# bhansconnect/burn-ppo

Hardware: AMD Instinct MI355X
Metric: env-steps/sec (rollout+GAE+PPO update) at 1/2/4/8 MI355X; steps-to-475-return CartPole (higher is better)
Workload: dtype f32

## Files before the change

### burn-ppo_amd/csrc/k_update.hip

```cpp
#include <algorithm>
#include <cstdlib>
#include "bppo_internal.h"
#include "bppo_mlp64.h"

namespace bppo {

constexpr int STAT_BLOCKS = 1024;

enum { M_PL = 0, M_VL, M_H, M_KL, M_CF, M_V, M_R, M_VE, M_VE2, M_VEMAX, M_N, NUM_M };

constexpr int ADAM_CHUNK = 4096;
struct AdamTensor { int off, len; float c1, c2; };
struct AdamArgs {
    float *params, *grad, *m1, *m2;
    double *part;
    AdamTensor t[32];
    int blk0[33];
    int nt;
    float lr, max_norm, eps, inv_world;
};
constexpr int SLAB_GROUPS = 32;

struct MbArgs {
    const float *obs, *logp, *adv, *ret, *val;
// ... 431 lines not shown
            float lh = 0.0f, vv = 0.0f;
            const float *hr = B.T2 + c * RS;
            const float2 *pv = S.PV[h];
#pragma unroll 16
            for (int k = 0; k < H; k++) {
                const float hk = hr[k];
                const float2 w = pv[k];
                lh = __builtin_fmaf(hk, w.x, lh);
                vv = __builtin_fmaf(hk, w.y, vv);
            }
            const float lx = __shfl_xor(lh, 32, 64);
            const float l0 = h ? lx : lh, l1 = h ? lh : lx;
            MB_STAMP(9);
            const float lg0 = __fadd_rn(l0, S.bp[0]), lg1 = __fadd_rn(l1, S.bp[1]), v = __fadd_rn(vv, S.bv[0]);
            const float mx = lg0 > lg1 ? lg0 : lg1;
            const float eh = S.expf(__fsub_rn(h ? lg1 : lg0, mx));
            const float eo = __shfl_xor(eh, 32, 64);
            const float e0 = h ? eo : eh, e1 = h ? eh : eo;
            const float lse = S.logf(__fadd_rn(e0, e1));
            const float ls0 = __fsub_rn(__fsub_rn(lg0, mx), lse);
            const float ls1 = __fsub_rn(__fsub_rn(lg1, mx), lse);
            const float ph = S.expf(h ? ls1 : ls0);
            const float po = __shfl_xor(ph, 32, 64);
            const float p0 = h ? po : ph, p1 = h ? ph : po;
          if (h == 0) {
            const float An = __fdiv_rn(__fsub_rn(A, mean), denom);
            const float Hn = -__fadd_rn(__fmul_rn(p0, ls0), __fmul_rn(p1, ls1));
            const float newlp = a == 1 ? ls1 : ls0;
            const float log_ratio = __fsub_rn(newlp, olp);
            const float ratio = S.expf(log_ratio);
            const float na = -An;
            const float pl1 = __fmul_rn(na, ratio);
            const float rc = ratio < g.lo ? g.lo : (ratio > g.hi ? g.hi : ratio);
            const float pl2 = __fmul_rn(na, rc);
            const bool rhs = pl1 < pl2;
            const float pl = rhs ? pl2 : pl1;
            float vl, dvl;
            if (g.clip_value) {
                const float dlt = __fsub_rn(v, ov);
                const float dc = dlt < -g.ceps ? -g.ceps : (dlt > g.ceps ? g.ceps : dlt);
                const float vc = __fadd_rn(ov, dc);
                const float q1 = __fmul_rn(__fsub_rn(v, R), __fsub_rn(v, R));
                const float q2 = __fmul_rn(__fsub_rn(vc, R), __fsub_rn(vc, R));
                if (q1 < q2) { vl = q2; dvl = (dlt >= -g.ceps && dlt <= g.ceps) ? 2.0f * __fsub_rn(vc, R) : 0.0f; }
                else { vl = q1; dvl = 2.0f * __fsub_rn(v, R); }
            } else {
                vl = __fmul_rn(__fsub_rn(v, R), __fsub_rn(v, R));
                dvl = 2.0f * __fsub_rn(v, R);
            }
            const float g_ratio = (!rhs || (ratio >= g.lo && ratio <= g.hi)) ? -An * g.inv_mb : 0.0f;
            const float g_lr = g_ratio * ratio;
            const float ec = g.ent_coef * g.inv_mb;
            float dl0 = g_lr * ((a == 0 ? 1.0f : 0.0f) - p0) + ec * p0 * (ls0 + Hn);
            float dl1 = g_lr * ((a == 1 ? 1.0f : 0.0f) - p1) + ec * p1 * (ls1 + Hn);
            float dv = g.value_coef * 0.5f * g.inv_mb * dvl;
            if (!valid) { dl0 = dl1 = dv = 0.0f; }
            else {
                const float ve = fabsf(__fsub_rn(v, R));
                m_pl += pl; m_vl += vl; m_h += Hn; m_kl += (ratio - 1.0f) - log_ratio;
                m_cf += fabsf(ratio - 1.0f) > g.ceps ? 1.0f : 0.0f;
                m_v += v; m_r += R; m_ve += ve; m_ve2 += ve * ve; m_vemax = fmaxf(m_vemax, ve);
                m_n += 1.0f;
            }
            gbp0 += dl0; gbp1 += dl1; gbv += dv;
            B.dl[c * 4 + 0] = dl0; B.dl[c * 4 + 1] = dl1; B.dl[c * 4 + 2] = dv; B.dl[c * 4 + 3] = 0.0f;
          }
        }
        wave_sync();
        MB_STAMP(10);
        MB_STAMP(4);
#pragma unroll 4
        for (int q = 0; q < 16; q++) {
            const int row = cd_row(q, h);
            const float d0 = B.dl[row * 4], d1 = B.dl[row * 4 + 1], dvr = B.dl[row * 4 + 2];
#pragma unroll
            for (int ct = 0; ct < 2; ct++) {
                const float hv = B.T2[row * RS + c + 32 * ct];
                gP0[ct] = __builtin_fmaf(hv, d0, gP0[ct]);
                gP1[ct] = __builtin_fmaf(hv, d1, gP1[ct]);
                gV[ct] = __builtin_fmaf(hv, dvr, gV[ct]);
            }
        }
#pragma unroll
        for (int ct = 0; ct < 2; ct++)
#pragma unroll
            for (int q = 0; q < 16; q++) acc[ct][q] = 0.0f;
        {
            const float a0 = B.dl[c * 4 + h], a1 = B.dl[c * 4 + 2 + h];
#pragma unroll
            for (int ct = 0; ct < 2; ct++) {
                acc[ct] = __builtin_amdgcn_mfma_f32_32x32x2f32(a0, h ? wpk1[ct] : wpk0[ct], acc[ct], 0, 0, 0);
                acc[ct] = __builtin_amdgcn_mfma_f32_32x32x2f32(a1, h ? 0.0f : wvk[ct], acc[ct], 0, 0, 0);
            }
        }
#pragma unroll
        for (int q = 0; q < 16; q++) {
#pragma unroll
            for (int ct = 0; ct < 2; ct++) {
                const int ad = cd_row(q, h) * RS + c + 32 * ct;
                const float dz = B.T2[ad] > 0.0f ? acc[ct][q] : 0.0f;
                gb1[ct] += dz;
                B.T2[ad] = dz;
            }
            if ((q & 3) == 3) __builtin_amdgcn_sched_barrier(0);
        }
        wave_sync();
        MB_STAMP(5);
#pragma unroll
        for (int jt = 0; jt < 2; jt++)
#pragma unroll
            for (int q = 0; q < 16; q++) acc[jt][q] = 0.0f;
        __builtin_amdgcn_s_setprio(3);
#pragma unroll 4
        for (int s2 = 0; s2 < 16; s2++) {
#pragma unroll
            for (int u = 0; u < 2; u++) {
                const int s = 2 * s2 + u;
                const float av = B.T2[c * RS + 2 * s + h];
                const float bw0 = S.W1[c * RS + 2 * s + h], bw1 = S.W1[(c + 32) * RS + 2 * s + h];
                acc[0] = __builtin_amdgcn_mfma_f32_32x32x2f32(av, bw0, acc[0], 0, 0, 0);
                acc[1] = __builtin_amdgcn_mfma_f32_32x32x2f32(av, bw1, acc[1], 0, 0, 0);
            }
            const int rr = (2 * s2 + h) * RS;
            const float a0 = B.T1[rr + c], a1 = B.T1[rr + c + 32];
            const float z0 = B.T2[rr + c], z1 = B.T2[rr + c + 32];
            dW1[0][0] = __builtin_amdgcn_mfma_f32_32x32x2f32(a0, z0, dW1[0][0], 0, 0, 0);
            dW1[0][1] = __builtin_amdgcn_mfma_f32_32x32x2f32(a0, z1, dW1[0][1], 0, 0, 0);
            dW1[1][0] = __builtin_amdgcn_mfma_f32_32x32x2f32(a1, z0, dW1[1][0], 0, 0, 0);
            dW1[1][1] = __builtin_amdgcn_mfma_f32_32x32x2f32(a1, z1, dW1[1][1], 0, 0, 0);
        }
        __builtin_amdgcn_s_setprio(0);
        MB_STAMP(6);
#pragma unroll
        for (int q = 0; q < 16; q++) {
            const int row = cd_row(q, h);
            float xr[5];
#pragma unroll
            for (int d = 0; d < 5; d++) xr[d] = B.X[row * 5 + d];
#pragma unroll
            for (int jt = 0; jt < 2; jt++) {
                const float dzv = B.T1[row * RS + c + 32 * jt] > 0.0f ? acc[jt][q] : 0.0f;
                gb0[jt] += dzv;
#pragma unroll
                for (int d = 0; d < 5; d++) gW0[d][jt] = __builtin_fmaf(xr[d], dzv, gW0[d][jt]);
            }
            if ((q & 3) == 3) __builtin_amdgcn_sched_barrier(0);
        }
        wave_sync();
        MB_STAMP(7);
    }
#pragma unroll
    for (int ct = 0; ct < 2; ct++) {
        gb0[ct] += __shfl_xor(gb0[ct], 32, 64); gb1[ct] += __shfl_xor(gb1[ct], 32, 64);
        gP0[ct] += __shfl_xor(gP0[ct], 32, 64); gP1[ct] += __shfl_xor(gP1[ct], 32, 64);
        gV[ct] += __shfl_xor(gV[ct], 32, 64);
#pragma unroll
        for (int d = 0; d < 5; d++) gW0[d][ct] += __shfl_xor(gW0[d][ct], 32, 64);
    }
    const int W_ = g.np + NUM_M;
    __syncthreads();
    float *row = smem + (size_t)wv * W_;
    if (h == 0) {
#pragma unroll
        for (int ct = 0; ct < 2; ct++) {
            const int k = c + 32 * ct;
#pragma unroll
            for (int d = 0; d < 5; d++) row[O.w0 + d * H + k] = gW0[d][ct];
            row[O.b0 + k] = gb0[ct];
            row[O.b1 + k] = gb1[ct];
            row[O.wp + 2 * k] = gP0[ct];
            row[O.wp + 2 * k + 1] = gP1[ct];
            row[O.wv + k] = gV[ct];
        }
    }
#pragma unroll
    for (int it = 0; it < 2; it++)
#pragma unroll
        for (int jt = 0; jt < 2; jt++)
#pragma unroll
            for (int q = 0; q < 16; q++)
                row[O.w1 + ((q & 3) + 8 * (q >> 2) + 4 * h + 32 * it) * H + c + 32 * jt] = dW1[it][jt][q];
    const float s_bp0 = wave_sum(gbp0), s_bp1 = wave_sum(gbp1), s_bv = wave_sum(gbv);
    const float s_pl = wave_sum(m_pl), s_vl = wave_sum(m_vl), s_h = wave_sum(m_h);
    const float s_kl = wave_sum(m_kl), s_cf = wave_sum(m_cf), s_v = wave_sum(m_v);
    const float s_r = wave_sum(m_r), s_ve = wave_sum(m_ve), s_ve2 = wave_sum(m_ve2);
    const float s_mx = wave_max(m_vemax), s_n = wave_sum(m_n);
    if (lane == 0) {
        row[O.bp] = s_bp0; row[O.bp + 1] = s_bp1; row[O.bv] = s_bv;
        float *mm = row + g.np;
        mm[M_PL] = s_pl; mm[M_VL] = s_vl; mm[M_H] = s_h; mm[M_KL] = s_kl; mm[M_CF] = s_cf;
        mm[M_V] = s_v; mm[M_R] = s_r; mm[M_VE] = s_ve; mm[M_VE2] = s_ve2; mm[M_VEMAX] = s_mx;
        mm[M_N] = s_n;
    }
    __syncthreads();
    for (int p = tid; p < W_; p += blockDim.x) {
        float acc = smem[p];
        if (p == g.np + M_VEMAX) {
            for (int w = 1; w < WAVES; w++) acc = fmaxf(acc, smem[(size_t)w * W_ + p]);
        } else {
            for (int w = 1; w < WAVES; w++) acc += smem[(size_t)w * W_ + p];
        }
        g.slab[(size_t)blockIdx.x * W_ + p] = acc;
    }
#ifdef BPPO_MB_STAMPS
    MB_STAMP(8);
    if (lane == 0)
        for (int k = 0; k < MB_NSEG; k++) g.stamps[(size_t)gwave * MB_NSEG + k] = st_acc[k];
#endif
}

namespace mmf {
constexpr int H = 64, TR = 32, WS = 68;
typedef __bf16 bf16x8_t __attribute__((ext_vector_type(8)));
typedef short s16x4_t __attribute__((ext_vector_type(4)));
typedef short s16x8_t __attribute__((ext_vector_type(8)));
struct Params {
    uint64_t exp2tab[32];
    double linvc[16], llogc[16];
    float W0[6 * H];
    float b1[H];
    float4 Wh[H];
    float bp[2], bv[2];
    float2 PV[2][H];
    __bf16 W1[3][H * H];
    __device__ __forceinline__ float expf(float x) const { return bppo_math::expf_glibc_tab(x, exp2tab); }
    __device__ __forceinline__ float logf(float x) const { return bppo_math::logf_glibc_tab(x, linvc, llogc); }
};
constexpr int MET_STRIDE = 20;
template <bool EXACT_FWD>
struct Wave {
    float X[TR * 5];
    union {
        float T[TR * WS];
        __bf16 Z[EXACT_FWD ? 4 : 3 * H * TR];
    };
    float dl[TR * 4];
    float met[TR * MET_STRIDE];
};
enum { MT_PL = 0, MT_VL, MT_H, MT_KL, MT_CF, MT_V, MT_R, MT_VE, MT_VE2, MT_VEMAX, MT_N, MT_BP0, MT_BP1, MT_BV };
constexpr int WAVES = 8;
constexpr size_t W1F_BYTES = H * H * sizeof(float);
template <bool EXACT_FWD>
constexpr size_t lds_tiles() { return sizeof(Params) + (EXACT_FWD ? W1F_BYTES : 0) + WAVES * sizeof(Wave<EXACT_FWD>); }
static_assert(lds_tiles<false>() <= 160 * 1024 && lds_tiles<true>() <= 160 * 1024,
              "split minibatch kernel LDS over the gfx950 limit");
static_assert(sizeof(Params) % 16 == 0 && offsetof(Params, W1) % 16 == 0 && sizeof(Wave<false>) % 16 == 0 &&
              sizeof(Wave<true>) % 16 == 0, "LDS images 16-B aligned");
__device__ __forceinline__ int w1_swz(int j1) { return (((j1 >> 1) & 1) << 2) | (((j1 >> 2) & 1) << 1) | ((j1 >> 3) & 1); }
__device__ __forceinline__ int w1_at(int j1, int j2) { return j1 * H + ((((j2 >> 3) ^ w1_swz(j1)) << 3) | (j2 & 7)); }
__device__ __forceinline__ int z_swz(int j2) { return ((j2 >> 2) & 7) ^ (((j2 >> 1) & 1) << 2); }
__device__ __forceinline__ int z_at(int j2, int row) { return j2 * TR + ((((row >> 2) ^ z_swz(j2)) << 2) | (row & 3)); }
__device__ __forceinline__ s16x4_t lds_tr4(const __bf16 *p) {
    return __builtin_amdgcn_ds_read_tr16_b64_v4i16((__attribute__((address_space(3))) s16x4_t *)p);
}
__device__ __forceinline__ bf16x8_t cat8(s16x4_t lo, s16x4_t hi) {
    return __builtin_bit_cast(bf16x8_t, (s16x8_t)__builtin_shufflevector(lo, hi, 0, 1, 2, 3, 4, 5, 6, 7));
}
struct Split8 { bf16x8_t p[3]; };
typedef __bf16 bf16x2_t __attribute__((ext_vector_type(2)));
__device__ __forceinline__ uint32_t pk_bf16(float a, float b) {
    uint32_t u = __builtin_bit_cast(uint32_t, bf16x2_t{(__bf16)a, (__bf16)b});
    asm("" : "+v"(u));
    return u;
}
union Pieces8 { bf16x8_t v; uint32_t u[4]; };
__device__ __forceinline__ Split8 split8(const float (&x)[8]) {
#ifdef BPPO_SPLIT8_SCALAR
    Split8 t;
#pragma unroll
    for (int j = 0; j < 8; j++) {
        const __bf16 a = (__bf16)x[j];
        const float r = x[j] - (float)a;
        const __bf16 b = (__bf16)r;
        t.p[0][j] = a; t.p[1][j] = b; t.p[2][j] = (__bf16)(r - (float)b);
    }
    return t;
#endif
    Pieces8 p0, p1, p2;
#pragma unroll
    for (int j = 0; j < 4; j++) {
        const float xa = x[2 * j], xb = x[2 * j + 1];
        const uint32_t A = pk_bf16(xa, xb);
        const float ra = xa - __uint_as_float(A << 16), rb = xb - __uint_as_float(A & 0xffff0000u);
        const uint32_t B = pk_bf16(ra, rb);
        const float sa = ra - __uint_as_float(B << 16), sb = rb - __uint_as_float(B & 0xffff0000u);
        p0.u[j] = A; p1.u[j] = B; p2.u[j] = pk_bf16(sa, sb);
    }
    Split8 s;
    s.p[0] = p0.v; s.p[1] = p1.v; s.p[2] = p2.v;
    return s;
}
__device__ __forceinline__ float relu_bits(float v) {
    const int b = __float_as_int(v);
    return __int_as_float(b > 0 ? b : 0);
}
__device__ __forceinline__ void mfma6(f32x16_t &acc, const Split8 &a, const Split8 &b) {
    acc = __builtin_amdgcn_mfma_f32_32x32x16_bf16(a.p[2], b.p[0], acc, 0, 0, 0);
    acc = __builtin_amdgcn_mfma_f32_32x32x16_bf16(a.p[1], b.p[1], acc, 0, 0, 0);
    acc = __builtin_amdgcn_mfma_f32_32x32x16_bf16(a.p[0], b.p[2], acc, 0, 0, 0);
    acc = __builtin_amdgcn_mfma_f32_32x32x16_bf16(a.p[1], b.p[0], acc, 0, 0, 0);
    acc = __builtin_amdgcn_mfma_f32_32x32x16_bf16(a.p[0], b.p[1], acc, 0, 0, 0);
    acc = __builtin_amdgcn_mfma_f32_32x32x16_bf16(a.p[0], b.p[0], acc, 0, 0, 0);
}
__device__ __forceinline__ Split8 w1_row_pieces(const __bf16 (*W1)[H * H], int j1, int j2) {
    Split8 s;
    const int off = w1_at(j1, j2);
#pragma unroll
    for (int p = 0; p < 3; p++) s.p[p] = *reinterpret_cast<const bf16x8_t *>(W1[p] + off);
    return s;
}
__device__ __forceinline__ Split8 w1_tr_pieces(const __bf16 (*W1)[H * H], int base, const int (&off)[2]) {
    Split8 s;
#pragma unroll
    for (int p = 0; p < 3; p++) s.p[p] = cat8(lds_tr4(W1[p] + base + off[0]), lds_tr4(W1[p] + base + off[1]));
    return s;
}
template <bool EXACT_FWD>
__device__ __forceinline__ void load_params_split(Params &S, float *W1f, const float *__restrict__ P) {
    constexpr CpOffsets O = cp_offsets<64, 2>();
    for (int i = threadIdx.x; i < 6 * H; i += blockDim.x) S.W0[i] = i < 5 * H ? P[O.w0 + i] : P[O.b0 + i - 5 * H];
    for (int t = threadIdx.x; t < H * H / 8; t += blockDim.x) {
        const int j1 = t >> 3, j2 = (t & 7) * 8;
        float w[8];
#pragma unroll
        for (int j = 0; j < 8; j++) w[j] = P[O.w1 + 8 * t + j];
        const Split8 sp = split8(w);
        const int off = w1_at(j1, j2);
#pragma unroll
        for (int p = 0; p < 3; p++) *reinterpret_cast<bf16x8_t *>(S.W1[p] + off) = sp.p[p];
        if (EXACT_FWD) {
#pragma unroll
            for (int j = 0; j < 8; j++) W1f[8 * t + j] = w[j];
        }
    }
    for (int i = threadIdx.x; i < H; i += blockDim.x) {
        S.b1[i] = P[O.b1 + i];
        S.Wh[i] = make_float4(P[O.wp + 2 * i], P[O.wp + 2 * i + 1], P[O.wv + i], 0.0f);
        if (EXACT_FWD) {
            S.PV[0][i] = make_float2(P[O.wp + 2 * i], P[O.wv + i]);
            S.PV[1][i] = make_float2(P[O.wp + 2 * i + 1], P[O.wv + i]);
        }
    }
    if (threadIdx.x < 32) S.exp2tab[threadIdx.x] = bppo_math::kExp2fTab[threadIdx.x];
    if (threadIdx.x < 16) {
        S.linvc[threadIdx.x] = bppo_math::kLogfInvc[threadIdx.x];
        S.llogc[threadIdx.x] = bppo_math::kLogfLogc[threadIdx.x];
    }
    if (threadIdx.x < 2) S.bp[threadIdx.x] = P[O.bp + threadIdx.x];
    if (threadIdx.x == 0) S.bv[0] = P[O.bv];
}
}

template <bool EXACT_FWD>
__global__ void __launch_bounds__(512, 2) k_minibatch_split(MbArgs g) {
    using namespace mmf;
    using mmb::cd_row;
    constexpr CpOffsets O = cp_offsets<64, 2>();
    extern __shared__ __attribute__((aligned(16))) float smem[];
    Params &S = *reinterpret_cast<Params *>(smem);
    float *W1f = smem + sizeof(Params) / 4;
    const int tid = threadIdx.x, lane = tid & 63, wv = tid >> 6;
    Wave<EXACT_FWD> &B = reinterpret_cast<Wave<EXACT_FWD> *>(smem + (sizeof(Params) + (EXACT_FWD ? W1F_BYTES : 0)) / 4)[wv];
    load_params_split<EXACT_FWD>(S, W1f, g.params);
    __syncthreads();
#ifdef BPPO_MB_STAMPS
    unsigned long long st_acc[MB_NSEG] = {}, st_prev;
    asm volatile("s_memtime %0\n\ts_waitcnt lgkmcnt(0)" : "=s"(st_prev)::"memory");
#endif

    const int c = lane & 31, h = lane >> 5;
    const int gwave = blockIdx.x * WAVES + wv, nwaves = gridDim.x * WAVES;
    const float mean = g.mb_stats[0], denom = g.mb_stats[1] + 1e-8f;
    int w1tr[2][2];
    {
        const int q = (lane >> 2) & 3, p = lane & 3, gq = (lane >> 4) & 1;
#pragma unroll
        for (int ct = 0; ct < 2; ct++)
#pragma unroll
            for (int e = 0; e < 2; e++) w1tr[ct][e] = w1_at(4 * h + 8 * e + q, 32 * ct + 16 * gq + 4 * p);
    }
    f32x16_t dW1[2][2];
#pragma unroll
    for (int i = 0; i < 2; i++)
#pragma unroll
        for (int j = 0; j < 2; j++)
#pragma unroll
            for (int q = 0; q < 16; q++) dW1[i][j][q] = 0.0f;
    float gW0[5][2], gb0[2] = {0, 0}, gb1[2] = {0, 0}, gP0[2] = {0, 0}, gP1[2] = {0, 0}, gV[2] = {0, 0};
#pragma unroll
    for (int d = 0; d < 5; d++) gW0[d][0] = gW0[d][1] = 0.0f;
    if (h == 0) {
        float4 *mp = reinterpret_cast<float4 *>(B.met + c * MET_STRIDE);
        mp[0] = make_float4(0, 0, 0, 0); mp[1] = make_float4(0, 0, 0, 0);
        mp[2] = make_float4(0, -INFINITY, 0, 0); mp[3] = make_float4(0, 0, 0, 0);
    }

    const uint32_t stride = (uint32_t)nwaves * TR;
    auto idx_of = [&](uint32_t b) -> uint32_t {
        const uint32_t rr = b + c;
        return (h == 0 && rr < g.n) ? g.perm[g.start + rr] : 0xFFFFFFFFu;
    };
    RowData nxt;
    uint32_t idx_next = idx_of((uint32_t)gwave * TR + stride);
    nxt = load_row(g, idx_of((uint32_t)gwave * TR));
    __builtin_amdgcn_s_waitcnt(0);
    for (uint32_t base = (uint32_t)gwave * TR; base < g.n; base += stride) {
        const uint32_t r = base + c;
        const bool valid = h == 0 && r < g.n;
        const RowData cur = row_used(nxt, g.clip_value);
        int ln_ = lane;
        asm volatile("" : "+v"(ln_));
        const int c = ln_ & 31, h = ln_ >> 5;
        const uint32_t idx_after = idx_of(base + 2 * stride);
        nxt = load_row(g, idx_next);
        idx_next = idx_after;
        const int a = cur.a;
        const float olp = cur.olp, A = cur.A, R = cur.R, ov = cur.ov;
        if (h == 0) {
#pragma unroll
            for (int d = 0; d < 5; d++) B.X[c * 5 + d] = cur.x(d);
        }
        wave_sync();
        MB_STAMP(0);
        float xs[3];
#pragma unroll
        for (int s = 0; s < 3; s++) xs[s] = (s == 2 && h == 1) ? 1.0f : B.X[c * 5 + 2 * s + h];
        f32x16_t h2[2];
#pragma unroll
        for (int ct = 0; ct < 2; ct++)
#pragma unroll
            for (int q = 0; q < 16; q++) h2[ct][q] = 0.0f;
        __builtin_amdgcn_s_setprio(3);
#pragma unroll
        for (int it = 0; it < 2; it++) {
            f32x16_t a1;
#pragma unroll
            for (int q = 0; q < 16; q++) a1[q] = 0.0f;
#pragma unroll
            for (int s = 0; s < 3; s++)
                a1 = __builtin_amdgcn_mfma_f32_32x32x2f32(S.W0[(2 * s + h) * H + c + 32 * it], xs[s], a1, 0, 0, 0);
            if (EXACT_FWD) {
#pragma unroll
                for (int q = 0; q < 16; q++) B.T[(cd_row(q, h) + 32 * it) * TR + c] = relu_bits(a1[q]);
                continue;
            }
#pragma unroll
            for (int s2 = 0; s2 < 2; s2++) {
                float v8[8];
#pragma unroll
                for (int j = 0; j < 8; j++) v8[j] = relu_bits(a1[8 * s2 + j]);
                const Split8 Af = split8(v8);
#pragma unroll
                for (int ct = 0; ct < 2; ct++)
                    mfma6(h2[ct], Af, w1_tr_pieces(S.W1, (32 * it + 16 * s2) * H, w1tr[ct]));
                __builtin_amdgcn_sched_barrier(0);
            }
        }
        if (EXACT_FWD) {
            wave_sync();
#pragma unroll 4
            for (int s = 0; s < 32; s++) {
                const float av = B.T[(2 * s + h) * TR + c];
                const float bv0 = W1f[(2 * s + h) * H + c], bv1 = W1f[(2 * s + h) * H + c + 32];
                h2[0] = __builtin_amdgcn_mfma_f32_32x32x2f32(av, bv0, h2[0], 0, 0, 0);
                h2[1] = __builtin_amdgcn_mfma_f32_32x32x2f32(av, bv1, h2[1], 0, 0, 0);
            }
        }
        __builtin_amdgcn_s_setprio(0);
        MB_STAMP(1);
        if (EXACT_FWD) wave_sync();
#pragma unroll
        for (int ct = 0; ct < 2; ct++)
#pragma unroll
            for (int q = 0; q < 16; q++) {
                const float v = h2[ct][q] + S.b1[c + 32 * ct];
                B.T[cd_row(q, h) * WS + c + 32 * ct] = relu_bits(v);
            }
        wave_sync();
        MB_STAMP(2);
        float l0, l1, vv;
        if (EXACT_FWD) {
            float lh = 0.0f, vc = 0.0f;
            const float *hr = B.T + c * WS;
            const float2 *pv = S.PV[h];
#pragma unroll 2
            for (int k = 0; k < H; k += 4) {
                const float4 x = *reinterpret_cast<const float4 *>(hr + k);
                const float xs4[4] = {x.x, x.y, x.z, x.w};
#pragma unroll
                for (int u = 0; u < 4; u++) {
                    const float2 w = pv[k + u];
                    lh = __builtin_fmaf(xs4[u], w.x, lh);
                    vc = __builtin_fmaf(xs4[u], w.y, vc);
                }
            }
            const float lx = __shfl_xor(lh, 32, 64);
            l0 = h ? lx : lh; l1 = h ? lh : lx; vv = vc;
        } else {
            float pa[3] = {0, 0, 0}, pb[3] = {0, 0, 0};
            const float *hr = B.T + c * WS + 32 * h;
#pragma unroll
            for (int k = 0; k < 32; k += 4) {
                const float4 x = *reinterpret_cast<const float4 *>(hr + k);
                const float4 w0 = S.Wh[32 * h + k], w1 = S.Wh[32 * h + k + 1];
                const float4 w2 = S.Wh[32 * h + k + 2], w3 = S.Wh[32 * h + k + 3];
                pa[0] = __builtin_fmaf(x.x, w0.x, pa[0]); pa[1] = __builtin_fmaf(x.x, w0.y, pa[1]); pa[2] = __builtin_fmaf(x.x, w0.z, pa[2]);
                pb[0] = __builtin_fmaf(x.y, w1.x, pb[0]); pb[1] = __builtin_fmaf(x.y, w1.y, pb[1]); pb[2] = __builtin_fmaf(x.y, w1.z, pb[2]);
                pa[0] = __builtin_fmaf(x.z, w2.x, pa[0]); pa[1] = __builtin_fmaf(x.z, w2.y, pa[1]); pa[2] = __builtin_fmaf(x.z, w2.z, pa[2]);
                pb[0] = __builtin_fmaf(x.w, w3.x, pb[0]); pb[1] = __builtin_fmaf(x.w, w3.y, pb[1]); pb[2] = __builtin_fmaf(x.w, w3.z, pb[2]);
            }
            float t0 = pa[0] + pb[0], t1 = pa[1] + pb[1], t2 = pa[2] + pb[2];
            t0 += __shfl_xor(t0, 32, 64); t1 += __shfl_xor(t1, 32, 64); t2 += __shfl_xor(t2, 32, 64);
            l0 = t0; l1 = t1; vv = t2;
        }
        MB_STAMP(3);
        {
            const float lg0 = __fadd_rn(l0, S.bp[0]), lg1 = __fadd_rn(l1, S.bp[1]), v = __fadd_rn(vv, S.bv[0]);
            const float mx = lg0 > lg1 ? lg0 : lg1;
            const float eh = S.expf(__fsub_rn(h ? lg1 : lg0, mx));
            const float eo = __shfl_xor(eh, 32, 64);
            const float e0 = h ? eo : eh, e1 = h ? eh : eo;
            const float lse = S.logf(__fadd_rn(e0, e1));
            const float ls0 = __fsub_rn(__fsub_rn(lg0, mx), lse);
            const float ls1 = __fsub_rn(__fsub_rn(lg1, mx), lse);
            const float ph = S.expf(h ? ls1 : ls0);
            const float po = __shfl_xor(ph, 32, 64);
            const float p0 = h ? po : ph, p1 = h ? ph : po;
          if (h == 0) {
            const float An = __fdiv_rn(__fsub_rn(A, mean), denom);
            const float Hn = -__fadd_rn(__fmul_rn(p0, ls0), __fmul_rn(p1, ls1));
            const float newlp = a == 1 ? ls1 : ls0;
            const float log_ratio = __fsub_rn(newlp, olp);
            const float ratio = S.expf(log_ratio);
            const float na = -An;
            const float pl1 = __fmul_rn(na, ratio);
            const float rc = ratio < g.lo ? g.lo : (ratio > g.hi ? g.hi : ratio);
            const float pl2 = __fmul_rn(na, rc);
            const bool rhs = pl1 < pl2;
            const float pl = rhs ? pl2 : pl1;
            float vl, dvl;
            if (g.clip_value) {
                const float dlt = __fsub_rn(v, ov);
                const float dc = dlt < -g.ceps ? -g.ceps : (dlt > g.ceps ? g.ceps : dlt);
                const float vc = __fadd_rn(ov, dc);
                const float q1 = __fmul_rn(__fsub_rn(v, R), __fsub_rn(v, R));
                const float q2 = __fmul_rn(__fsub_rn(vc, R), __fsub_rn(vc, R));
                if (q1 < q2) { vl = q2; dvl = (dlt >= -g.ceps && dlt <= g.ceps) ? 2.0f * __fsub_rn(vc, R) : 0.0f; }
                else { vl = q1; dvl = 2.0f * __fsub_rn(v, R); }
            } else {
                vl = __fmul_rn(__fsub_rn(v, R), __fsub_rn(v, R));
                dvl = 2.0f * __fsub_rn(v, R);
            }
            const float g_ratio = (!rhs || (ratio >= g.lo && ratio <= g.hi)) ? -An * g.inv_mb : 0.0f;
            const float g_lr = g_ratio * ratio;
            const float ec = g.ent_coef * g.inv_mb;
            float dl0 = g_lr * ((a == 0 ? 1.0f : 0.0f) - p0) + ec * p0 * (ls0 + Hn);
            float dl1 = g_lr * ((a == 1 ? 1.0f : 0.0f) - p1) + ec * p1 * (ls1 + Hn);
            float dv = g.value_coef * 0.5f * g.inv_mb * dvl;
            if (!valid) { dl0 = dl1 = dv = 0.0f; }
            else {
                const float ve = fabsf(__fsub_rn(v, R));
                float4 *mp = reinterpret_cast<float4 *>(B.met + c * MET_STRIDE);
                float4 m0 = mp[0], m1 = mp[1], m2 = mp[2], m3 = mp[3];
                m0.x += pl; m0.y += vl; m0.z += Hn; m0.w += (ratio - 1.0f) - log_ratio;
                m1.x += fabsf(ratio - 1.0f) > g.ceps ? 1.0f : 0.0f;
                m1.y += v; m1.z += R; m1.w += ve; m2.x += ve * ve; m2.y = fmaxf(m2.y, ve);
                m2.z += 1.0f; m2.w += dl0; m3.x += dl1; m3.y += dv;
                mp[0] = m0; mp[1] = m1; mp[2] = m2; mp[3] = m3;
            }
            *reinterpret_cast<float4 *>(B.dl + c * 4) = make_float4(dl0, dl1, dv, 0.0f);
          }
        }
        wave_sync();
        MB_STAMP(4);
#pragma unroll 4
        for (int q = 0; q < 16; q++) {
            const int row = cd_row(q, h);
            const float4 d = *reinterpret_cast<const float4 *>(B.dl + row * 4);
#pragma unroll
            for (int ct = 0; ct < 2; ct++) {
                const float hv = B.T[row * WS + c + 32 * ct];
                gP0[ct] = __builtin_fmaf(hv, d.x, gP0[ct]);
                gP1[ct] = __builtin_fmaf(hv, d.y, gP1[ct]);
                gV[ct] = __builtin_fmaf(hv, d.z, gV[ct]);
            }
        }
        f32x16_t acc[2];
#pragma unroll
        for (int ct = 0; ct < 2; ct++)
#pragma unroll
            for (int q = 0; q < 16; q++) acc[ct][q] = 0.0f;
        {
            const float a0 = B.dl[c * 4 + h], a1 = B.dl[c * 4 + 2 + h];
#pragma unroll
            for (int ct = 0; ct < 2; ct++) {
                const float4 w = S.Wh[c + 32 * ct];
                acc[ct] = __builtin_amdgcn_mfma_f32_32x32x2f32(a0, h ? w.y : w.x, acc[ct], 0, 0, 0);
                acc[ct] = __builtin_amdgcn_mfma_f32_32x32x2f32(a1, h ? 0.0f : w.z, acc[ct], 0, 0, 0);
            }
        }
        if (EXACT_FWD) {
#pragma unroll
            for (int q = 0; q < 16; q++) {
#pragma unroll
                for (int ct = 0; ct < 2; ct++) {
                    const int ad = cd_row(q, h) * WS + c + 32 * ct;
                    const float dz = B.T[ad] > 0.0f ? acc[ct][q] : 0.0f;
                    gb1[ct] += dz;
                    B.T[ad] = dz;
                }
                if ((q & 3) == 3) __builtin_amdgcn_sched_barrier(0);
            }
        } else {
#pragma unroll
            for (int q = 0; q < 16; q++)
#pragma unroll
                for (int ct = 0; ct < 2; ct++) {
                    acc[ct][q] = B.T[cd_row(q, h) * WS + c + 32 * ct] > 0.0f ? acc[ct][q] : 0.0f;
                    gb1[ct] += acc[ct][q];
                }
            wave_sync();
#pragma unroll
            for (int s2 = 0; s2 < 2; s2++)
#pragma unroll
                for (int t = 0; t < 2; t++) {
                    float z[8];
#pragma unroll
                    for (int j = 0; j < 8; j++) z[j] = acc[t][8 * s2 + j];
                    const Split8 P = split8(z);
#pragma unroll
                    for (int p = 0; p < 3; p++) {
                        const uint4 u = __builtin_bit_cast(uint4, P.p[p]);
                        *reinterpret_cast<uint2 *>(B.Z + p * H * TR + z_at(c + 32 * t, 16 * s2 + 4 * h)) = make_uint2(u.x, u.y);
                        *reinterpret_cast<uint2 *>(B.Z + p * H * TR + z_at(c + 32 * t, 16 * s2 + 8 + 4 * h)) = make_uint2(u.z, u.w);
                    }
                    __builtin_amdgcn_sched_barrier(0);
                }
        }
        MB_STAMP(5);
        __builtin_amdgcn_s_setprio(3);
        f32x16_t h1[2];
#pragma unroll
        for (int jt = 0; jt < 2; jt++)
#pragma unroll
            for (int q = 0; q < 16; q++) h1[jt][q] = 0.0f;
#pragma unroll
        for (int s = 0; s < 3; s++) {
            const float xv = (s == 2 && h == 1) ? 1.0f : B.X[c * 5 + 2 * s + h];
#pragma unroll
            for (int jt = 0; jt < 2; jt++)
                h1[jt] = __builtin_amdgcn_mfma_f32_32x32x2f32(xv, S.W0[(2 * s + h) * H + c + 32 * jt], h1[jt], 0, 0, 0);
        }
        uint32_t m1 = 0;
#pragma unroll
        for (int jt = 0; jt < 2; jt++)
#pragma unroll
            for (int q = 0; q < 16; q++) {
                h1[jt][q] = relu_bits(h1[jt][q]);
                const uint32_t hb = __float_as_uint(h1[jt][q]);
                m1 |= (hb < 1u ? hb : 1u) << (q + 16 * jt);
            }
        MB_STAMP(6);
#pragma unroll
        for (int s2 = 0; s2 < 2; s2++) {
            Split8 Bz[2];
#pragma unroll
            for (int t = 0; t < 2; t++) {
                if (EXACT_FWD) {
                    float z[8];
#pragma unroll
                    for (int j = 0; j < 8; j++) z[j] = B.T[cd_row(8 * s2 + j, h) * WS + c + 32 * t];
                    Bz[t] = split8(z);
                } else {
#pragma unroll
                    for (int p = 0; p < 3; p++) {
                        const uint2 lo = *reinterpret_cast<const uint2 *>(B.Z + p * H * TR + z_at(c + 32 * t, 16 * s2 + 4 * h));
                        const uint2 hi = *reinterpret_cast<const uint2 *>(B.Z + p * H * TR + z_at(c + 32 * t, 16 * s2 + 8 + 4 * h));
                        Bz[t].p[p] = __builtin_bit_cast(bf16x8_t, make_uint4(lo.x, lo.y, hi.x, hi.y));
                    }
                }
            }
#pragma unroll
            for (int it = 0; it < 2; it++) {
                float u[8];
#pragma unroll
                for (int j = 0; j < 8; j++) u[j] = h1[it][8 * s2 + j];
                const Split8 Ah = split8(u);
#pragma unroll
                for (int jt = 0; jt < 2; jt++) mfma6(dW1[it][jt], Ah, Bz[jt]);
                __builtin_amdgcn_sched_barrier(0);
            }
        }
        wave_sync();
        MB_STAMP(7);
        f32x16_t dz1[2];
#pragma unroll
        for (int ct = 0; ct < 2; ct++)
#pragma unroll
            for (int q = 0; q < 16; q++) dz1[ct][q] = 0.0f;
#pragma unroll
        for (int ks = 0; ks < 4; ks++) {
            Split8 Az;
            if (EXACT_FWD) {
                const float *zr = B.T + c * WS + 16 * ks + 8 * h;
                const float4 z0 = *reinterpret_cast<const float4 *>(zr), z1 = *reinterpret_cast<const float4 *>(zr + 4);
                const float zz[8] = {z0.x, z0.y, z0.z, z0.w, z1.x, z1.y, z1.z, z1.w};
                Az = split8(zz);
            } else {
                const int q = (lane >> 2) & 3, pp = lane & 3, gq = (lane >> 4) & 1;
#pragma unroll
                for (int p = 0; p < 3; p++)
                    Az.p[p] = cat8(lds_tr4(B.Z + p * H * TR + z_at(16 * ks + 8 * h + q, 16 * gq + 4 * pp)),
                                   lds_tr4(B.Z + p * H * TR + z_at(16 * ks + 8 * h + 4 + q, 16 * gq + 4 * pp)));
            }
#pragma unroll
            for (int ct = 0; ct < 2; ct++)
                mfma6(dz1[ct], Az, w1_row_pieces(S.W1, c + 32 * ct, 16 * ks + 8 * h));
            __builtin_amdgcn_sched_barrier(0);
        }
        __builtin_amdgcn_s_setprio(0);
        MB_STAMP(8);
#pragma unroll
        for (int q = 0; q < 16; q++) {
            const int row = cd_row(q, h);
            float xr[5];
#pragma unroll
            for (int d = 0; d < 5; d++) xr[d] = B.X[row * 5 + d];
#pragma unroll
            for (int jt = 0; jt < 2; jt++) {
                const int mk = (int)(m1 << (31 - (q + 16 * jt))) >> 31;
                const float dzv = __int_as_float(__float_as_int(dz1[jt][q]) & mk);
                gb0[jt] += dzv;
#pragma unroll
                for (int d = 0; d < 5; d++) gW0[d][jt] = __builtin_fmaf(xr[d], dzv, gW0[d][jt]);
            }
            if ((q & 3) == 3) __builtin_amdgcn_sched_barrier(0);
        }
        wave_sync();
        MB_STAMP(9);
    }
#pragma unroll
    for (int ct = 0; ct < 2; ct++) {
        gb0[ct] += __shfl_xor(gb0[ct], 32, 64); gb1[ct] += __shfl_xor(gb1[ct], 32, 64);
        gP0[ct] += __shfl_xor(gP0[ct], 32, 64); gP1[ct] += __shfl_xor(gP1[ct], 32, 64);
        gV[ct] += __shfl_xor(gV[ct], 32, 64);
#pragma unroll
        for (int d = 0; d < 5; d++) gW0[d][ct] += __shfl_xor(gW0[d][ct], 32, 64);
    }
    float mt[14];
#pragma unroll
    for (int k = 0; k < 14; k++) mt[k] = h == 0 ? B.met[c * MET_STRIDE + k] : (k == MT_VEMAX ? -INFINITY : 0.0f);
    const int W_ = g.np + NUM_M;
    __syncthreads();
    float *row = smem + (size_t)wv * W_;
    if (h == 0) {
#pragma unroll
        for (int ct = 0; ct < 2; ct++) {
            const int k = c + 32 * ct;
#pragma unroll
            for (int d = 0; d < 5; d++) row[O.w0 + d * H + k] = gW0[d][ct];
            row[O.b0 + k] = gb0[ct];
            row[O.b1 + k] = gb1[ct];
            row[O.wp + 2 * k] = gP0[ct];
            row[O.wp + 2 * k + 1] = gP1[ct];
            row[O.wv + k] = gV[ct];
        }
    }
#pragma unroll
    for (int it = 0; it < 2; it++)
#pragma unroll
        for (int jt = 0; jt < 2; jt++)
#pragma unroll
            for (int q = 0; q < 16; q++)
                row[O.w1 + ((q & 3) + 8 * (q >> 2) + 4 * h + 32 * it) * H + c + 32 * jt] = dW1[it][jt][q];
    float st[14];
#pragma unroll
    for (int k = 0; k < 14; k++) st[k] = k == MT_VEMAX ? wave_max(mt[k]) : wave_sum(mt[k]);
    if (lane == 0) {
        row[O.bp] = st[MT_BP0]; row[O.bp + 1] = st[MT_BP1]; row[O.bv] = st[MT_BV];
        float *mm = row + g.np;
        static_assert(MT_PL == M_PL && MT_VEMAX == M_VEMAX && MT_N == M_N, "metric slots");
#pragma unroll
        for (int k = 0; k <= MT_N; k++) mm[k] = st[k];
    }
    __syncthreads();
    for (int p = tid; p < W_; p += blockDim.x) {
        float a2 = smem[p];
        if (p == g.np + M_VEMAX) {
            for (int w = 1; w < WAVES; w++) a2 = fmaxf(a2, smem[(size_t)w * W_ + p]);
        } else {
            for (int w = 1; w < WAVES; w++) a2 += smem[(size_t)w * W_ + p];
        }
        g.slab[(size_t)blockIdx.x * W_ + p] = a2;
    }
#ifdef BPPO_MB_STAMPS
    MB_STAMP(10);
    if (lane == 0)
        for (int k = 0; k < MB_NSEG; k++) g.stamps[(size_t)gwave * MB_NSEG + k] = st_acc[k];
#endif
}

constexpr int SLAB1_COLS = 16;
__global__ void __launch_bounds__(SLAB1_COLS * SLAB_GROUPS) k_slab_reduce1(const float *__restrict__ slab, int rows,
                                                                           int width, float *__restrict__ grad,
                                                                           float *__restrict__ vemax_local) {
    __shared__ double part[SLAB_GROUPS][SLAB1_COLS];
    const int c = threadIdx.x % SLAB1_COLS, g = threadIdx.x / SLAB1_COLS;
    const int p = blockIdx.x * SLAB1_COLS + c;
    const bool live = p < width, is_max = p == width - NUM_M + M_VEMAX;
    const int per = (rows + SLAB_GROUPS - 1) / SLAB_GROUPS;
    if (live) {
        const int w0 = g * per, w1 = min(rows, w0 + per);
        double s = is_max ? -INFINITY : 0.0;
#pragma unroll 8
        for (int w = w0; w < w1; w++) {
            const double v = slab[(size_t)w * width + p];
            s = is_max ? fmax(s, v) : s + v;
        }
        part[g][c] = s;
    }
    __syncthreads();
    if (g == 0 && live) {
        double s = is_max ? -INFINITY : 0.0;
        for (int q = 0; q < SLAB_GROUPS; q++) s = is_max ? fmax(s, part[q][c]) : s + part[q][c];
        grad[p] = (float)s;
        if (is_max) *vemax_local = (float)s;
    }
}

__device__ __forceinline__ int adam_tensor_of(const AdamArgs &a, int b) {
    int t = 0;
    while (t + 1 < a.nt && a.blk0[t + 1] <= b) t++;
    return t;
}
__global__ void __launch_bounds__(256) k_adam_norm(AdamArgs a) {
    __shared__ double red[256];
    const int ti = adam_tensor_of(a, blockIdx.x);
    const AdamTensor T = a.t[ti];
    const int i0 = (blockIdx.x - a.blk0[ti]) * ADAM_CHUNK, i1 = min(T.len, i0 + ADAM_CHUNK);
    double ss = 0.0;
    for (int i = i0 + threadIdx.x; i < i1; i += blockDim.x) {
        const float gi = a.grad[T.off + i] * a.inv_world;
        ss += (double)gi * (double)gi;
    }
    red[threadIdx.x] = ss;
    __syncthreads();
    for (int st = 128; st > 0; st >>= 1) {
        if (threadIdx.x < st) red[threadIdx.x] += red[threadIdx.x + st];
        __syncthreads();
    }
    if (threadIdx.x == 0) a.part[blockIdx.x] = red[0];
}
__global__ void __launch_bounds__(256) k_adam(AdamArgs a) {
    __shared__ double tot;
    const int ti = adam_tensor_of(a, blockIdx.x);
    const AdamTensor T = a.t[ti];
    if (threadIdx.x == 0) {
        double s = 0.0;
        for (int b = a.blk0[ti]; b < a.blk0[ti + 1]; b++) s += a.part[b];
        tot = s;
    }
    __syncthreads();
    const int i0 = (blockIdx.x - a.blk0[ti]) * ADAM_CHUNK, i1 = min(T.len, i0 + ADAM_CHUNK);
    const float norm = (float)sqrt(tot);
    const float scale = norm > a.max_norm ? __fdiv_rn(a.max_norm, norm) : 1.0f;
    const bool clip = norm > a.max_norm;
    const float b1 = 0.9f, b2 = 0.999f, f1 = 1.0f - 0.9f, f2 = 1.0f - 0.999f;
    for (int i = i0 + threadIdx.x; i < i1; i += blockDim.x) {
        float gi = a.grad[T.off + i] * a.inv_world;
        if (clip) gi = __fmul_rn(gi, scale);
        const float m1 = __fadd_rn(__fmul_rn(a.m1[T.off + i], b1), __fmul_rn(gi, f1));
        const float m2 = __fadd_rn(__fmul_rn(a.m2[T.off + i], b2), __fmul_rn(__fmul_rn(gi, gi), f2));
        a.m1[T.off + i] = m1;
        a.m2[T.off + i] = m2;
        const float m1c = __fdiv_rn(m1, T.c1), m2c = __fdiv_rn(m2, T.c2);
        const float upd = __fdiv_rn(m1c, __fadd_rn(sqrtf(m2c), a.eps));
        a.params[T.off + i] = __fsub_rn(a.params[T.off + i], __fmul_rn(upd, a.lr));
    }
}

constexpr int ADAM1_THREADS = 1024;
__global__ void __launch_bounds__(ADAM1_THREADS) k_adam1(AdamArgs a, const float *gtail, const float *mb_stats,
                                                         int nm, float *metric_dst) {
    __shared__ double red[256];
    const AdamTensor T = a.t[blockIdx.x];
    if (threadIdx.x < 256) {
        double ss = 0.0;
#pragma unroll 4
        for (int i = threadIdx.x; i < T.len; i += 256) {
            const float gi = a.grad[T.off + i] * a.inv_world;
            ss += (double)gi * (double)gi;
        }
        red[threadIdx.x] = ss;
    }
    __syncthreads();
    for (int st = 128; st > 0; st >>= 1) {
        if (threadIdx.x < st) red[threadIdx.x] += red[threadIdx.x + st];
        __syncthreads();
    }
    const double tot = red[0];
    const float norm = (float)sqrt(tot);
    const float scale = norm > a.max_norm ? __fdiv_rn(a.max_norm, norm) : 1.0f;
    const bool clip = norm > a.max_norm;
    const float b1 = 0.9f, b2 = 0.999f, f1 = 1.0f - 0.9f, f2 = 1.0f - 0.999f;
#pragma unroll 2
    for (int i = threadIdx.x; i < T.len; i += ADAM1_THREADS) {
        float gi = a.grad[T.off + i] * a.inv_world;
        if (clip) gi = __fmul_rn(gi, scale);
        const float m1 = __fadd_rn(__fmul_rn(a.m1[T.off + i], b1), __fmul_rn(gi, f1));
        const float m2 = __fadd_rn(__fmul_rn(a.m2[T.off + i], b2), __fmul_rn(__fmul_rn(gi, gi), f2));
        a.m1[T.off + i] = m1;
        a.m2[T.off + i] = m2;
        const float m1c = __fdiv_rn(m1, T.c1), m2c = __fdiv_rn(m2, T.c2);
        const float upd = __fdiv_rn(m1c, __fadd_rn(sqrtf(m2c), a.eps));
        a.params[T.off + i] = __fsub_rn(a.params[T.off + i], __fmul_rn(upd, a.lr));
    }
    if (blockIdx.x == 0 && metric_dst) {
        const int i = threadIdx.x;
        if (i < nm) metric_dst[i] = gtail[i == GRAD_VEMAX ? GRAD_VEMAX_LOCAL : i];
        else if (i < nm + 4) metric_dst[i] = mb_stats[i - nm];
    }
}

__global__ void __launch_bounds__(256) k_ev(size_t n, const float *val, const float *ret, const float *valid,
                                             double *part) {
    __shared__ double sh[4][256];
    double s[4] = {0, 0, 0, 0};
    for (size_t i = blockIdx.x * blockDim.x + threadIdx.x; i < n; i += (size_t)gridDim.x * blockDim.x) {
        if (valid && !(valid[i] > 0.5f)) continue;
        const double R = ret[i], res = (double)(ret[i] - val[i]);
        s[0] += R; s[1] += R * R; s[2] += res; s[3] += res * res;
    }
    for (int k = 0; k < 4; k++) sh[k][threadIdx.x] = s[k];
    __syncthreads();
    for (int st = 128; st > 0; st >>= 1) {
        if (threadIdx.x < st)
            for (int k = 0; k < 4; k++) sh[k][threadIdx.x] += sh[k][threadIdx.x + st];
        __syncthreads();
    }
    if (threadIdx.x == 0)
        for (int k = 0; k < 4; k++) part[blockIdx.x * 4 + k] = sh[k][0];
}

constexpr int ADV_THREADS = 1024, ADV_U = 4;
__global__ void __launch_bounds__(ADV_THREADS) k_adv_epoch(const float *__restrict__ adv,
                                                           const uint32_t *__restrict__ perm, EpochSplit sp,
                                                           uint32_t C, double *part) {
    __shared__ double red[ADV_THREADS / 64][2][4];
    const uint32_t i0 = blockIdx.x * C, i1 = min(sp.B, i0 + C);
    const uint32_t m0 = mb_of(i0, sp);
    double s[2] = {0.0, 0.0}, q[2] = {0.0, 0.0};
    float mn[2] = {INFINITY, INFINITY}, mx[2] = {-INFINITY, -INFINITY};
    for (uint32_t b = i0 + threadIdx.x; b < i1; b += ADV_THREADS * ADV_U) {
        uint32_t pi[ADV_U];
        float a[ADV_U];
#pragma unroll
        for (int k = 0; k < ADV_U; k++) pi[k] = perm[min(b + k * ADV_THREADS, i1 - 1)];
#pragma unroll
        for (int k = 0; k < ADV_U; k++) a[k] = adv[pi[k]];
#pragma unroll
        for (int k = 0; k < ADV_U; k++) {
            const uint32_t i = b + k * ADV_THREADS;
            if (i >= i1) continue;
            const double d = (double)a[k];
            if (mb_of(i, sp) != m0) { s[1] += d; q[1] += d * d; mn[1] = fminf(mn[1], a[k]); mx[1] = fmaxf(mx[1], a[k]); }
            else { s[0] += d; q[0] += d * d; mn[0] = fminf(mn[0], a[k]); mx[0] = fmaxf(mx[0], a[k]); }
        }
    }
    const int lane = threadIdx.x & 63, w = threadIdx.x >> 6;
#pragma unroll
    for (int k = 0; k < 2; k++) {
        double x = s[k], y = q[k];
        float u = mn[k], v = mx[k];
#pragma unroll
        for (int o = 32; o > 0; o >>= 1) {
            x += __shfl_xor(x, o, 64); y += __shfl_xor(y, o, 64);
            u = fminf(u, __shfl_xor(u, o, 64)); v = fmaxf(v, __shfl_xor(v, o, 64));
        }
        if (lane == 0) { red[w][k][0] = x; red[w][k][1] = y; red[w][k][2] = u; red[w][k][3] = v; }
    }
    __syncthreads();
    if (threadIdx.x < 2) {
        const int k = threadIdx.x;
        double x = 0.0, y = 0.0, u = INFINITY, v = -INFINITY;
        for (int ww = 0; ww < ADV_THREADS / 64; ww++) {
            x += red[ww][k][0]; y += red[ww][k][1]; u = fmin(u, red[ww][k][2]); v = fmax(v, red[ww][k][3]);
        }
        double *o = part + ((size_t)blockIdx.x * 2 + k) * 4;
        o[0] = x; o[1] = y; o[2] = u; o[3] = v;
    }
}
__global__ void __launch_bounds__(256) k_adv_epoch_final(const double *part, int nblk, uint32_t C, EpochSplit sp,
                                                         float *stats) {
    __shared__ double ss[256], sq[256], smn[256], smx[256];
    const uint32_t m = blockIdx.x;
    double s = 0.0, q = 0.0, mn = INFINITY, mx = -INFINITY;
    for (int b = threadIdx.x; b < nblk; b += blockDim.x) {
        const uint32_t m0 = mb_of((uint32_t)b * C, sp);
        if (m != m0 && m != m0 + 1) continue;
        const double *o = part + ((size_t)b * 2 + (m != m0)) * 4;
        s += o[0]; q += o[1]; mn = fmin(mn, o[2]); mx = fmax(mx, o[3]);
    }
    ss[threadIdx.x] = s; sq[threadIdx.x] = q; smn[threadIdx.x] = mn; smx[threadIdx.x] = mx;
    __syncthreads();
    for (int st = 128; st > 0; st >>= 1) {
        if (threadIdx.x < st) {
            ss[threadIdx.x] += ss[threadIdx.x + st]; sq[threadIdx.x] += sq[threadIdx.x + st];
            smn[threadIdx.x] = fmin(smn[threadIdx.x], smn[threadIdx.x + st]);
            smx[threadIdx.x] = fmax(smx[threadIdx.x], smx[threadIdx.x + st]);
        }
        __syncthreads();
    }
    if (threadIdx.x != 0) return;
    const double n = (double)(sp.base + (m < sp.rem ? 1u : 0u));
    const double mean = ss[0] / n;
    stats[m * 4 + 0] = (float)mean;
    stats[m * 4 + 1] = n > 1.0 ? sqrtf((float)(fmax(sq[0] - ss[0] * mean, 0.0) / (n - 1.0))) : NAN;
    stats[m * 4 + 2] = (float)smn[0];
    stats[m * 4 + 3] = (float)smx[0];
}

// ... 257 lines not shown
```

Measured before the change: 777.8 million.

## Software-pipeline split-bf16 MFMA loops with prefetch and sched_group_barrier interleaving

Restructures the forward layer-1 and backward dW1/dz1 MFMA loops so the next fragment's LDS loads and bf16 split conversion are issued while the current six-MFMA group runs. Explicit sched_group_barrier patterns interleave MFMA, DS-read and VALU instructions. The relu/mask computation is folded into fragment construction, and a wave_sync is moved ahead of the backward stage. The goal is to hide LDS latency and conversion VALU work behind matrix ops, at the cost of more live registers and possible occupancy or spill pressure.

After: 751.6 million. 3.4% lower.

```diff
diff --git a/burn-ppo_amd/csrc/k_update.hip b/burn-ppo_amd/csrc/k_update.hip
--- a/burn-ppo_amd/csrc/k_update.hip
+++ b/burn-ppo_amd/csrc/k_update.hip
@@ -757,6 +757,17 @@
     acc = __builtin_amdgcn_mfma_f32_32x32x16_bf16(a.p[0], b.p[1], acc, 0, 0, 0);
     acc = __builtin_amdgcn_mfma_f32_32x32x16_bf16(a.p[0], b.p[0], acc, 0, 0, 0);
 }
+template <int ND, int NV>
+__device__ __forceinline__ void issue1() {
+    __builtin_amdgcn_sched_group_barrier(0x008, 1, 0);
+    if constexpr (ND > 0) __builtin_amdgcn_sched_group_barrier(0x100, ND, 0);
+    if constexpr (NV > 0) __builtin_amdgcn_sched_group_barrier(0x002, NV, 0);
+}
+template <int ND, int NV>
+__device__ __forceinline__ void issue6() {
+    issue1<ND, NV>(); issue1<ND, NV>(); issue1<ND, NV>();
+    issue1<0, NV>(); issue1<0, NV>(); issue1<0, NV>();
+}
 __device__ __forceinline__ Split8 w1_row_pieces(const __bf16 (*W1)[H * H], int j1, int j2) {
     Split8 s;
     const int off = w1_at(j1, j2);
@@ -886,29 +897,58 @@
 #pragma unroll
             for (int q = 0; q < 16; q++) h2[ct][q] = 0.0f;
         __builtin_amdgcn_s_setprio(3);
-#pragma unroll
-        for (int it = 0; it < 2; it++) {
-            f32x16_t a1;
-#pragma unroll
-            for (int q = 0; q < 16; q++) a1[q] = 0.0f;
+        if (EXACT_FWD) {
+#pragma unroll
+            for (int it = 0; it < 2; it++) {
+                f32x16_t a1;
+#pragma unroll
+                for (int q = 0; q < 16; q++) a1[q] = 0.0f;
+#pragma unroll
+                for (int s = 0; s < 3; s++)
+                    a1 = __builtin_amdgcn_mfma_f32_32x32x2f32(S.W0[(2 * s + h) * H + c + 32 * it], xs[s], a1, 0, 0, 0);
+#pragma unroll
+                for (int q = 0; q < 16; q++) B.T[(cd_row(q, h) + 32 * it) * TR + c] = relu_bits(a1[q]);
+            }
+        } else {
+            f32x16_t a1[2];
+#pragma unroll
+            for (int it = 0; it < 2; it++)
+#pragma unroll
+                for (int q = 0; q < 16; q++) a1[it][q] = 0.0f;
 #pragma unroll
             for (int s = 0; s < 3; s++)
-                a1 = __builtin_amdgcn_mfma_f32_32x32x2f32(S.W0[(2 * s + h) * H + c + 32 * it], xs[s], a1, 0, 0, 0);
-            if (EXACT_FWD) {
-#pragma unroll
-                for (int q = 0; q < 16; q++) B.T[(cd_row(q, h) + 32 * it) * TR + c] = relu_bits(a1[q]);
-                continue;
-            }
-#pragma unroll
-            for (int s2 = 0; s2 < 2; s2++) {
+                a1[0] = __builtin_amdgcn_mfma_f32_32x32x2f32(S.W0[(2 * s + h) * H + c], xs[s], a1[0], 0, 0, 0);
+            Split8 Bw = w1_tr_pieces(S.W1, 0, w1tr[0]);
+            Split8 Af;
+            {
                 float v8[8];
 #pragma unroll
-                for (int j = 0; j < 8; j++) v8[j] = relu_bits(a1[8 * s2 + j]);
-                const Split8 Af = split8(v8);
-#pragma unroll
-                for (int ct = 0; ct < 2; ct++)
-                    mfma6(h2[ct], Af, w1_tr_pieces(S.W1, (32 * it + 16 * s2) * H, w1tr[ct]));
-                __builtin_amdgcn_sched_barrier(0);
+                for (int j = 0; j < 8; j++) v8[j] = relu_bits(a1[0][j]);
+                Af = split8(v8);
+            }
+            __builtin_amdgcn_sched_barrier(0);
+#pragma unroll
+            for (int i = 0; i < 4; i++) {
+                const Split8 Bw1 = w1_tr_pieces(S.W1, 16 * i * H, w1tr[1]);
+                mfma6(h2[0], Af, Bw);
+                Split8 An = Af;
+                if (i < 3) {
+                    float v8[8];
+#pragma unroll
+                    for (int j = 0; j < 8; j++) v8[j] = relu_bits(a1[(i + 1) >> 1][8 * ((i + 1) & 1) + j]);
+                    An = split8(v8);
+                    Bw = w1_tr_pieces(S.W1, 16 * (i + 1) * H, w1tr[0]);
+                }
+                mfma6(h2[1], Af, Bw1);
+                Af = An;
+                issue6<2, 5>();
+                issue6<2, 5>();
+                if (i == 0) {
+#pragma unroll
+                    for (int s = 0; s < 3; s++)
+                        a1[1] = __builtin_amdgcn_mfma_f32_32x32x2f32(S.W0[(2 * s + h) * H + c + 32], xs[s], a1[1], 0, 0, 0);
+                    issue1<0, 0>(); issue1<0, 0>(); issue1<0, 0>();
+                }
             }
         }
         if (EXACT_FWD) {
@@ -1092,6 +1132,7 @@
                     __builtin_amdgcn_sched_barrier(0);
                 }
         }
+        wave_sync();
         MB_STAMP(5);
         __builtin_amdgcn_s_setprio(3);
         f32x16_t h1[2];
@@ -1107,71 +1148,103 @@
                 h1[jt] = __builtin_amdgcn_mfma_f32_32x32x2f32(xv, S.W0[(2 * s + h) * H + c + 32 * jt], h1[jt], 0, 0, 0);
         }
         uint32_t m1 = 0;
-#pragma unroll
-        for (int jt = 0; jt < 2; jt++)
-#pragma unroll
-            for (int q = 0; q < 16; q++) {
-                h1[jt][q] = relu_bits(h1[jt][q]);
-                const uint32_t hb = __float_as_uint(h1[jt][q]);
-                m1 |= (hb < 1u ? hb : 1u) << (q + 16 * jt);
-            }
         MB_STAMP(6);
-#pragma unroll
-        for (int s2 = 0; s2 < 2; s2++) {
-            Split8 Bz[2];
-#pragma unroll
-            for (int t = 0; t < 2; t++) {
-                if (EXACT_FWD) {
-                    float z[8];
-#pragma unroll
-                    for (int j = 0; j < 8; j++) z[j] = B.T[cd_row(8 * s2 + j, h) * WS + c + 32 * t];
-                    Bz[t] = split8(z);
-                } else {
-#pragma unroll
-                    for (int p = 0; p < 3; p++) {
-                        const uint2 lo = *reinterpret_cast<const uint2 *>(B.Z + p * H * TR + z_at(c + 32 * t, 16 * s2 + 4 * h));
-                        const uint2 hi = *reinterpret_cast<const uint2 *>(B.Z + p * H * TR + z_at(c + 32 * t, 16 * s2 + 8 + 4 * h));
-                        Bz[t].p[p] = __builtin_bit_cast(bf16x8_t, make_uint4(lo.x, lo.y, hi.x, hi.y));
-                    }
+        auto dz2_frag = [&](int s2, int t) -> Split8 {
+            Split8 f;
+            if (EXACT_FWD) {
+                float z[8];
+#pragma unroll
+                for (int j = 0; j < 8; j++) z[j] = B.T[cd_row(8 * s2 + j, h) * WS + c + 32 * t];
+                f = split8(z);
+            } else {
+#pragma unroll
+                for (int p = 0; p < 3; p++) {
+                    const uint2 lo = *reinterpret_cast<const uint2 *>(B.Z + p * H * TR + z_at(c + 32 * t, 16 * s2 + 4 * h));
+                    const uint2 hi = *reinterpret_cast<const uint2 *>(B.Z + p * H * TR + z_at(c + 32 * t, 16 * s2 + 8 + 4 * h));
+                    f.p[p] = __builtin_bit_cast(bf16x8_t, make_uint4(lo.x, lo.y, hi.x, hi.y));
                 }
             }
-#pragma unroll
-            for (int it = 0; it < 2; it++) {
-                float u[8];
-#pragma unroll
-                for (int j = 0; j < 8; j++) u[j] = h1[it][8 * s2 + j];
-                const Split8 Ah = split8(u);
-#pragma unroll
-                for (int jt = 0; jt < 2; jt++) mfma6(dW1[it][jt], Ah, Bz[jt]);
-                __builtin_amdgcn_sched_barrier(0);
-            }
-        }
-        wave_sync();
-        MB_STAMP(7);
-        f32x16_t dz1[2];
-#pragma unroll
-        for (int ct = 0; ct < 2; ct++)
-#pragma unroll
-            for (int q = 0; q < 16; q++) dz1[ct][q] = 0.0f;
-#pragma unroll
-        for (int ks = 0; ks < 4; ks++) {
-            Split8 Az;
+            return f;
+        };
+        auto h1_frag = [&](int i) -> Split8 {
+            float u[8];
+#pragma unroll
+            for (int j = 0; j < 8; j++) {
+                const int q = 8 * (i >> 1) + j;
+                u[j] = relu_bits(h1[i & 1][q]);
+                const uint32_t hb = __float_as_uint(u[j]);
+                m1 |= (hb < 1u ? hb : 1u) << (q + 16 * (i & 1));
+            }
+            return split8(u);
+        };
+        auto dz2_rows = [&](int ks) -> Split8 {
+            Split8 f;
             if (EXACT_FWD) {
                 const float *zr = B.T + c * WS + 16 * ks + 8 * h;
                 const float4 z0 = *reinterpret_cast<const float4 *>(zr), z1 = *reinterpret_cast<const float4 *>(zr + 4);
                 const float zz[8] = {z0.x, z0.y, z0.z, z0.w, z1.x, z1.y, z1.z, z1.w};
-                Az = split8(zz);
+                f = split8(zz);
             } else {
                 const int q = (lane >> 2) & 3, pp = lane & 3, gq = (lane >> 4) & 1;
 #pragma unroll
                 for (int p = 0; p < 3; p++)
-                    Az.p[p] = cat8(lds_tr4(B.Z + p * H * TR + z_at(16 * ks + 8 * h + q, 16 * gq + 4 * pp)),
-                                   lds_tr4(B.Z + p * H * TR + z_at(16 * ks + 8 * h + 4 + q, 16 * gq + 4 * pp)));
-            }
-#pragma unroll
-            for (int ct = 0; ct < 2; ct++)
-                mfma6(dz1[ct], Az, w1_row_pieces(S.W1, c + 32 * ct, 16 * ks + 8 * h));
+                    f.p[p] = cat8(lds_tr4(B.Z + p * H * TR + z_at(16 * ks + 8 * h + q, 16 * gq + 4 * pp)),
+                                  lds_tr4(B.Z + p * H * TR + z_at(16 * ks + 8 * h + 4 + q, 16 * gq + 4 * pp)));
+            }
+            return f;
+        };
+        Split8 Az, Bw[2];
+        {
+            constexpr int ND = EXACT_FWD ? 3 : 2, NV = EXACT_FWD ? 8 : 6;
+            Split8 Bz[2] = {dz2_frag(0, 0), dz2_frag(0, 1)};
+            Split8 Bn[2];
+            Split8 Ah = h1_frag(0);
             __builtin_amdgcn_sched_barrier(0);
+#pragma unroll
+            for (int i = 0; i < 4; i++) {
+                Split8 An = Ah;
+                mfma6(dW1[i & 1][0], Ah, Bz[0]);
+                if (i < 2) Bn[i] = dz2_frag(1, i);
+                if (i < 3) An = h1_frag(i + 1);
+                mfma6(dW1[i & 1][1], Ah, Bz[1]);
+                Ah = An;
+                if (i == 1) { Bz[0] = Bn[0]; Bz[1] = Bn[1]; }
+                if (i == 3) {
+                    Az = dz2_rows(0);
+                    Bw[0] = w1_row_pieces(S.W1, c, 8 * h);
+                    Bw[1] = w1_row_pieces(S.W1, c + 32, 8 * h);
+                }
+                if (i < 2) { issue6<ND, NV>(); issue6<0, NV>(); }
+                else if (i == 2) { issue6<0, NV>(); issue6<0, NV>(); }
+                else {
+                    issue1<2, NV>(); issue1<2, NV>(); issue1<2, NV>(); issue1<2, NV>(); issue1<2, NV>(); issue1<2, NV>();
+                    issue6<0, 0>();
+                }
+            }
+            __builtin_amdgcn_sched_barrier(0);
+        }
+        MB_STAMP(7);
+        f32x16_t dz1[2];
+#pragma unroll
+        for (int ct = 0; ct < 2; ct++)
+#pragma unroll
+            for (int q = 0; q < 16; q++) dz1[ct][q] = 0.0f;
+        {
+            constexpr int NV = EXACT_FWD ? 4 : 1;
+#pragma unroll
+            for (int ks = 0; ks < 4; ks++) {
+                Split8 An = Az, Bn0 = Bw[0], Bn1 = Bw[1];
+                mfma6(dz1[0], Az, Bw[0]);
+                if (ks < 3) {
+                    An = dz2_rows(ks + 1);
+                    Bn0 = w1_row_pieces(S.W1, c, 16 * (ks + 1) + 8 * h);
+                }
+                mfma6(dz1[1], Az, Bw[1]);
+                if (ks < 3) Bn1 = w1_row_pieces(S.W1, c + 32, 16 * (ks + 1) + 8 * h);
+                Az = An; Bw[0] = Bn0; Bw[1] = Bn1;
+                if (ks < 3) { issue6<3, NV>(); issue6<1, NV>(); }
+                else { issue6<0, 0>(); issue6<0, 0>(); }
+            }
         }
         __builtin_amdgcn_s_setprio(0);
         MB_STAMP(8);
```
